# jonH34400/3DBodyAnimation

Hardware: AMD Instinct MI355X
Metric: SMPL residual+Jacobian evals/sec (6890v, 10 beta, 24 joints) (higher is better)
Workload: dtype f64 residual/Jacobian; f32 mesh (f32 + split-bf16 MFMA blend); 1 GPU; C3: 256 independent frames per GPU, BODY_25 (14 FK joints + 11 vertex landmarks), opt-shape (per-frame beta, 86 cols), GMM prior on, 6890-vertex mesh on; frames_per_gpu=256, keypoints_per_frame=25, n_cols=86

## Files before the change

### 3dbodyanimation_amd/csrc/frame_part_inl.h

```cpp
#pragma once
#include <hip/hip_ext.h>

#include "bodyfit_device.h"
#include "priors_inl.h"

namespace bodyfit {
namespace {

__device__ __forceinline__ void store_through(double* p, double v) {
  __hip_atomic_store(p, v, __ATOMIC_RELAXED, __HIP_MEMORY_SCOPE_SYSTEM);
}
#ifndef BODYFIT_J_THROUGH
#define BODYFIT_J_THROUGH 1
#endif
template <bool kFused>
__device__ __forceinline__ void store_J(double* p, double v, int scope = 0) {
  if constexpr (kFused && !BODYFIT_J_THROUGH) *p = v;
  else if (scope == 1) store_f64_through(p, v);
  else if (scope == 2) *p = v;
  else store_through(p, v);
}


__device__ inline void mul33(const double* A, const double* B, double* C) {
#pragma unroll
  for (int r = 0; r < 3; ++r)
#pragma unroll
    for (int c = 0; c < 3; ++c) C[r * 3 + c] = A[r * 3] * B[c] + A[r * 3 + 1] * B[3 + c] + A[r * 3 + 2] * B[6 + c];
}
__device__ inline void mul33_bt(const double* A, const double* B, double* C) {
#pragma unroll
  for (int r = 0; r < 3; ++r)
#pragma unroll
    for (int c = 0; c < 3; ++c)
      C[r * 3 + c] = A[r * 3] * B[c * 3] + A[r * 3 + 1] * B[c * 3 + 1] + A[r * 3 + 2] * B[c * 3 + 2];
}
__device__ inline void mv3(const double* A, double x0, double x1, double x2, double* y) {
#pragma unroll
  for (int r = 0; r < 3; ++r) y[r] = A[r * 3] * x0 + A[r * 3 + 1] * x1 + A[r * 3 + 2] * x2;
}

__device__ void rodrigues_grad_k(double a0, double a1, double a2, int k, double* R, double* dRk) {
  const double th2 = a0 * a0 + a1 * a1 + a2 * a2;
  if (th2 > 2.220446049250313e-16) {
    const double th = sqrt(th2), ith = 1.0 / th;
    double sh, ch;
    sincos(0.5 * th, &sh, &ch);
    const double st = 2.0 * sh * ch, omc = 2.0 * sh * sh, ct = 1.0 - omc;
    const double w[3] = {a0 * ith, a1 * ith, a2 * ith};
    const double K[9] = {0, -w[2], w[1], w[2], 0, -w[0], -w[1], w[0], 0};
#pragma unroll
    for (int r = 0; r < 3; ++r)
#pragma unroll
      for (int c = 0; c < 3; ++c) R[r * 3 + c] = (r == c ? ct : 0.0) + st * K[r * 3 + c] + omc * w[r] * w[c];
    const double wk = (k == 0) ? w[0] : (k == 1 ? w[1] : w[2]);
    double dw[3];
#pragma unroll
    for (int i = 0; i < 3; ++i) dw[i] = ((i == k ? 1.0 : 0.0) - w[i] * wk) * ith;
    const double dK[9] = {0, -dw[2], dw[1], dw[2], 0, -dw[0], -dw[1], dw[0], 0};
#pragma unroll
    for (int r = 0; r < 3; ++r)
#pragma unroll
      for (int c = 0; c < 3; ++c)
        dRk[r * 3 + c] = (r == c ? -st * wk : 0.0) + ct * wk * K[r * 3 + c] + st * dK[r * 3 + c] +
                         st * wk * w[r] * w[c] + omc * (dw[r] * w[c] + w[r] * dw[c]);
  } else {
    R[0] = 1; R[1] = -a2; R[2] = a1;
    R[3] = a2; R[4] = 1; R[5] = -a0;
    R[6] = -a1; R[7] = a0; R[8] = 1;
#pragma unroll
    for (int i = 0; i < 9; ++i) dRk[i] = 0.0;
    if (k == 0) { dRk[5] = -1; dRk[7] = 1; }
    else if (k == 1) { dRk[2] = 1; dRk[6] = -1; }
    else { dRk[1] = -1; dRk[3] = 1; }
  }
}

__device__ inline double wave_sum(double v) {
#pragma unroll
  for (int off = 32; off > 0; off >>= 1) v += __shfl_down(v, off, 64);
  return v;
}

#ifdef BODYFIT_STAMPS
#define STAMP(i)                                                                              \
  do {                                                                                        \
    if (Pb.dbg && (threadIdx.x & 63) == 0) {                                                  \
      unsigned long long t_;                                                                  \
      asm volatile("s_memtime %0\n\ts_waitcnt lgkmcnt(0)" : "=s"(t_)::"memory");              \
      Pb.dbg[((size_t)f * 8 + (threadIdx.x >> 6)) * 16 + (i)] = t_;                  \
    }                                                                                         \
  } while (0)
#define STAMP_REAL(i)                                                                         \
  do {                                                                                        \
    if (Pb.dbg && (threadIdx.x & 63) == 0) {                                                  \
      unsigned long long t_;                                                                  \
      asm volatile("s_memrealtime %0\n\ts_waitcnt lgkmcnt(0)" : "=s"(t_)::"memory");          \
      Pb.dbg[((size_t)f * 8 + (threadIdx.x >> 6)) * 16 + (i)] = t_;                  \
    }                                                                                         \
  } while (0)
#else
#define STAMP(i)
#define STAMP_REAL(i)
#endif

constexpr int KC = 32;
constexpr int kThreads = 512;

constexpr int OFF_X = 0;
constexpr int OFF_R = OFF_X + 88;
constexpr int OFF_DR = OFF_R + 216;
constexpr int OFF_A = OFF_DR + 648;
constexpr int OFF_P = OFF_A + 216;
constexpr int OFF_O = OFF_P + 72;
constexpr int OFF_JC = OFF_O + 72;
constexpr int OFF_W = OFF_JC + 72;
constexpr int OFF_B = OFF_W + 624;
constexpr int OFF_FEAT = OFF_B + 720;
constexpr int OFF_CAM = OFF_FEAT + 208;
constexpr int OFF_KP = OFF_CAM + 40;
constexpr int OFF_TAB = OFF_KP + KC * 18;
constexpr int OFF_KPUV = OFF_TAB + 64;
constexpr int OFF_DS = OFF_KPUV + 2 * KC;
constexpr int OFF_SC = OFF_DS + 720;
constexpr int OFF_PART = OFF_SC + 720;
constexpr int OFF_T = OFF_PART + 128;
constexpr int OFF_CHAIN = OFF_T + 720;
constexpr int OFF_LM = OFF_CHAIN + 24;
constexpr int LM_VP = 0;
constexpr int LM_Q = 3;
constexpr int LM_A = 6;
constexpr int LM_X = 15;
constexpr int LM_W = 39;
constexpr int LM_J = 47;
constexpr int LM_NW = 51;
constexpr int LM_BETA = 52;
constexpr int LM_PD = 82;
constexpr int LM_STRIDE = 290;
constexpr int TAB_PARENT = 0;
constexpr int TAB_ANC = 24;
constexpr int TAB_KPID = 96;

struct FrameHead {
  const unsigned char* mtab;
  const unsigned char* ptab;
  const double* R0;
  int F, K;
  int dims;
};
static_assert(kMaxJoints < 64 && kMaxShape < 16 && kMaxLandmarks < 64 && 7 + 3 * (kMaxJoints - 1) + kMaxShape < 256,
              "FrameHead::dims: 6 + 4 + 6 + 8 bits for nJ, nS, nL, ncols; beta_stride (0 or nS) in 4");
__host__ __device__ inline int frame_head_dims(int nJ, int nS, int nL, int ncols, int use_shape, int beta_stride, int has_coef) {
  return nJ | (nS << 6) | (nL << 10) | (ncols << 16) | ((use_shape ? 1 : 0) << 24) | (beta_stride << 25) | ((has_coef ? 1 : 0) << 29);
}

struct FusedFrame {
  unsigned* flag;
  unsigned epoch;
  int j_scope;
};

template <bool kFused>
__device__ __forceinline__ void frame_sync() {
  if constexpr (kFused) asm volatile("s_waitcnt lgkmcnt(0)\n\ts_barrier" ::: "memory");
  else __syncthreads();
}

template <bool kFused>
__device__ __forceinline__ void store_operand16(void* p, uint4 v) {
  if constexpr (kFused) {
    typedef __attribute__((ext_vector_type(4))) unsigned int u32x4_;
    const u32x4_ x = {v.x, v.y, v.z, v.w};
    asm volatile("global_store_dwordx4 %0, %1, off sc1\n\ts_nop 1" ::"v"(p), "v"(x) : "memory");
  } else {
    *reinterpret_cast<uint4*>(p) = v;
  }
}

template <bool kFused>
__device__ __forceinline__ void frame_part(const DevModel& M, const DevProblem& Pb, const double* __restrict__ params,
                                           const double* __restrict__ beta, double* __restrict__ r_out,
                                           double* __restrict__ J_out, double* __restrict__ joints_out, const MeshCoef& mc,
                                           int want_jac, double* sm, int f, const FusedFrame& fu, const FrameHead& hd) {
  const int tid = threadIdx.x;
  const int lane = tid & 63, wave = tid >> 6;
  const int nJ = kFused ? (hd.dims & 63) : M.nJ, nS = kFused ? ((hd.dims >> 6) & 15) : M.nS, nL = kFused ? ((hd.dims >> 10) & 63) : M.nL;
  const int ncols = kFused ? ((hd.dims >> 16) & 255) : Pb.ncols;
  const int npose = 7 + 3 * (nJ - 1);
  const bool use_shape = kFused ? (((hd.dims >> 24) & 1) != 0) : (Pb.use_shape != 0);
  const int beta_stride = kFused ? ((hd.dims >> 25) & 15) : Pb.beta_stride;
  const unsigned char* const mtab = kFused ? hd.mtab : M.tabA;
  const unsigned char* const ptab = kFused ? hd.ptab : Pb.ptab;
  const int* const t_parent = reinterpret_cast<const int*>(mtab + kTabParent);
  const unsigned* const t_anc = reinterpret_cast<const unsigned*>(mtab + kTabAnc);
  const unsigned long long* const t_chain = reinterpret_cast<const unsigned long long*>(mtab + kTabChain);
  const int* const t_lm_woff = reinterpret_cast<const int*>(mtab + kTabLmWoff);
  const int* const t_lm_wj = reinterpret_cast<const int*>(mtab + kTabLmWj);
  const double* const t_lm_ww = reinterpret_cast<const double*>(mtab + kTabLmWw);
  const double* const t_lm_vt = reinterpret_cast<const double*>(mtab + kTabLmVt);
  const double* const t_lm_sd = reinterpret_cast<const double*>(mtab + kTabLmSd);
  const double* const t_dS = reinterpret_cast<const double*>(mtab + kTabDS);
  const double* const t_Sc = reinterpret_cast<const double*>(mtab + kTabSc);
  const double* const t_offset = reinterpret_cast<const double*>(mtab + kTabOffset);
  const double* const t_Jc0 = reinterpret_cast<const double*>(mtab + kTabJc0);
  const int t_F = kFused ? hd.F : Pb.F, t_K = kFused ? hd.K : Pb.K;
  const int* const t_kp_offset = reinterpret_cast<const int*>(ptab);
  const int* const t_kp_id = reinterpret_cast<const int*>(ptab + ptab_id_off(t_F));
  const double* const t_kp_uv = reinterpret_cast<const double*>(ptab + ptab_uv_off(t_F, t_K));
  const double* const t_R0 = kFused ? hd.R0 : Pb.R0;
  const int P = M.P;
  double* sx = sm + OFF_X;
  double* sR = sm + OFF_R;
  double* sdR = sm + OFF_DR;
  double* sA = sm + OFF_A;
  double* sP = sm + OFF_P;
  double* sO = sm + OFF_O;
  double* sJc = sm + OFF_JC;
  double* sW = sm + OFF_W;
  double* sB = sm + OFF_B;
  double* sFeat = sm + OFF_FEAT;
  double* sCam = sm + OFF_CAM;
  double* sKp = sm + OFF_KP;
  int* sTab = reinterpret_cast<int*>(sm + OFF_TAB);
  double* sKpUv = sm + OFF_KPUV;
  double* sDS = sm + OFF_DS;
  double* sSc = sm + OFF_SC;
  double* sPart = sm + OFF_PART;
  double* sLm = sm + OFF_LM;
  double* sT = sm + OFF_T;
  double* sLmSd = sLm + nL * LM_STRIDE;
  int* sParent = sTab + TAB_PARENT;
  unsigned* sAnc = reinterpret_cast<unsigned*>(sTab + TAB_ANC);
  int* sKpId = sTab + TAB_KPID;
  unsigned* sKpAnc = reinterpret_cast<unsigned*>(sTab + 48);
  unsigned long long* sChain = reinterpret_cast<unsigned long long*>(sm + OFF_CHAIN);

  STAMP_REAL(10);
  STAMP(0);
#ifdef BODYFIT_STAMPS
  if (Pb.dbg && tid == 0) {
    unsigned xcc;
    asm volatile("s_getreg_b32 %0, hwreg(HW_REG_XCC_ID)" : "=s"(xcc));
    Pb.dbg[((size_t)f * 8) * 16 + 9] = xcc & 0xf;
  }
#endif
  if constexpr (!kFused) {
    if (Pb.frame_flags && !(Pb.frame_flags[f] & Pb.frame_mask)) return;
  }
  constexpr int kLoaders = kThreads;
  constexpr bool loader = true;
  constexpr int kSdPasses = (kMaxLandmarks * 3 * kMaxShape + kThreads - 1) / kThreads;
  constexpr int kPasses = (720 + kLoaders - 1) / kLoaders;
  const bool coef_wave = kFused && wave == 5 && ((hd.dims >> 29) & 1) != 0;
  const int tj_c = min(tid, nJ - 1);
  const int par_in = t_parent[tj_c];
  const unsigned anc_in = t_anc[tj_c];
  const unsigned long long chain_in = t_chain[tj_c];
  const int nlw = nL * kMaxLmNnz, lw_i = min(tid, max(nlw, 1) - 1);
  const double lww_in = t_lm_ww[lw_i];
  const int lwj_in = t_lm_wj[lw_i];
  const int lwo_in = t_lm_woff[lw_i / kMaxLmNnz];
  const int nsd = nL * 3 * nS, nds = nJ * 3 * nS;
  double sd_in[kSdPasses], t0[kPasses], t1[kPasses];
#pragma unroll
  for (int u = 0; u < kSdPasses; ++u) sd_in[u] = t_lm_sd[min(tid + u * kThreads, max(nsd, 1) - 1)];
#pragma unroll
  for (int u = 0; u < kPasses; ++u) {
    const int i = min(tid + u * kLoaders, max(nds, 1) - 1);
    t0[u] = t_dS[i];
    t1[u] = t_Sc[i];
  }
  const int k_begin0 = t_kp_offset[f], nk0 = min(KC, t_kp_offset[f + 1] - k_begin0);
  const int o_i = tid - 128, v_row = tid - 256;
  const bool o_lane = tid >= 128 && o_i < nJ * 3, v_lane = tid >= 256 && v_row < nL * 3;
  double o_pre = 0.0, jc_pre = 0.0, vt_pre = 0.0;
  if (o_lane) { o_pre = t_offset[o_i]; jc_pre = t_Jc0[o_i]; }
  if (v_lane) vt_pre = t_lm_vt[v_row];
  const int cam_lane = tid - 384;
  const bool cam_on = cam_lane >= 0 && cam_lane < 36;
  double r0c0 = 0.0, r0c1 = 0.0, r0c2 = 0.0;
  if (cam_on) {
    const double* R0 = t_R0 + (size_t)f * 9;
    const int c = cam_lane % 3;
    r0c0 = R0[c]; r0c1 = R0[3 + c]; r0c2 = R0[6 + c];
  }
  double x_in = 0.0;
  const bool x_lane = tid >= 128 && tid - 128 < npose, b_lane = tid >= 224 && tid - 224 < nS;
  if (x_lane) x_in = params[(size_t)f * npose + tid - 128];
  if (b_lane) x_in = (use_shape && beta) ? beta[(size_t)f * beta_stride + tid - 224] : 0.0;
  int kp_id0 = 0;
  double kp_u0 = 0.0, kp_v0 = 0.0;
  if (loader) {
    kp_id0 = t_kp_id[k_begin0 + (tid & (KC - 1))];
    kp_u0 = t_kp_uv[2 * (size_t)(k_begin0 + (tid & (KC - 1)))];
    kp_v0 = t_kp_uv[2 * (size_t)(k_begin0 + (tid & (KC - 1))) + 1];
  }
  if (tid < nJ) { sParent[tid] = par_in; sAnc[tid] = anc_in; sChain[tid] = chain_in; }
  volatile int* sWalkDone = reinterpret_cast<volatile int*>(sPart + 104);
  if (tid == 0) *sWalkDone = 0;
  if (tid < nlw) {
    const int l = tid / kMaxLmNnz, i = tid % kMaxLmNnz;
    double* L = sLm + l * LM_STRIDE;
    L[LM_W + i] = lww_in;
    reinterpret_cast<int*>(L + LM_J)[i] = lwj_in;
    if (i == 0) L[LM_NW] = (double)lwo_in;
  }
#pragma unroll
  for (int u = 0; u < kSdPasses; ++u)
    if (tid + u * kThreads < nsd) sLmSd[tid + u * kThreads] = sd_in[u];
#pragma unroll
  for (int u = 0; u < kPasses; ++u) {
    const int i = tid + u * kLoaders;
    if (i < nds) { sDS[i] = t0[u]; sSc[i] = t1[u]; }
  }
  if (x_lane) sx[tid - 128] = x_in;
  if (b_lane) sx[npose + tid - 224] = x_in;
  frame_sync<kFused>();
  if (tid < nk0) {
    sTab[TAB_KPID + tid] = kp_id0;
    sKpUv[2 * tid] = kp_u0;
    sKpUv[2 * tid + 1] = kp_v0;
  }
  const double* sbeta = sx + npose;

  STAMP(1);
  if (tid < 3 * nJ) {
    const int jj = tid / 3, k = tid - 3 * jj;
    const double* aa = (jj == 0) ? (sx + 1) : (sx + 7 + 3 * (jj - 1));
    double R[9], dRk[9];
    rodrigues_grad_k(aa[0], aa[1], aa[2], k, R, dRk);
    if (k == 0) {
#pragma unroll
      for (int i = 0; i < 9; ++i) sR[jj * 9 + i] = R[i];
    }
#pragma unroll
    for (int i = 0; i < 9; ++i) sdR[jj * 27 + k * 9 + i] = dRk[i];
  }
  if (v_lane) {
    const int row = v_row;
    double sv[kMaxShape];
#pragma unroll
    for (int k = 0; k < kMaxShape; ++k) sv[k] = (use_shape && k < nS) ? sLmSd[row * nS + k] : 0.0;
    double acc = vt_pre;
#pragma unroll
    for (int k = 0; k < kMaxShape; ++k) acc += sv[k] * sbeta[min(k, nS > 0 ? nS - 1 : 0)];
    sPart[row] = acc;
  }
  if (coef_wave) {
    float* cf = reinterpret_cast<float*>(sW);
    const int nfeat = 9 * (nJ - 1);
    if (lane < nJ - 1) {
      const float a0 = (float)sx[7 + 3 * lane], a1 = (float)sx[8 + 3 * lane], a2 = (float)sx[9 + 3 * lane];
      const float th2 = a0 * a0 + a1 * a1 + a2 * a2;
      float st = 1.0f, omc = 0.0f, w0 = a0, w1 = a1, w2 = a2;
      if (th2 > 1e-20f) {
        const float ith = rsqrtf(th2), th = th2 * ith;
        float sh, ch;
        sincosf(0.5f * th, &sh, &ch);
        st = 2.0f * sh * ch; omc = 2.0f * sh * sh;
        w0 = a0 * ith; w1 = a1 * ith; w2 = a2 * ith;
      }
      const float on = Pb.pose_blend ? 1.0f : 0.0f;
      float* o = cf + 9 * lane;
      o[0] = on * (omc * (w0 * w0 - 1.0f)); o[1] = on * (omc * w0 * w1 - st * w2); o[2] = on * (omc * w0 * w2 + st * w1);
      o[3] = on * (omc * w1 * w0 + st * w2); o[4] = on * (omc * (w1 * w1 - 1.0f)); o[5] = on * (omc * w1 * w2 - st * w0);
      o[6] = on * (omc * w2 * w0 - st * w1); o[7] = on * (omc * w2 * w1 + st * w0); o[8] = on * (omc * (w2 * w2 - 1.0f));
    } else if (lane >= 32 && lane - 32 < 16 * kBlendKSteps - kPoseFeat) {
      const int i = lane - 32;
      cf[kPoseFeat + i] = (i < nS) ? (float)sbeta[i] : ((i == kMaxShape || i == kMaxShape + 1) ? 1.0f : 0.0f);
    }
    if (lane < 32)
      for (int k = nfeat + lane; k < kPoseFeat; k += 32) cf[k] = 0.0f;
  }
  if (o_lane) {
    const int i = o_i;
    double o = o_pre, jc = jc_pre;
    if (use_shape) {
      for (int k = 0; k < nS; ++k) {
        o += sDS[i * nS + k] * sbeta[k];
        jc += sSc[i * nS + k] * sbeta[k];
      }
    }
    sO[i] = (i < 3) ? 0.0 : o;
    if (i < 3) sPart[100 + i] = o;
    sJc[i] = jc;
  }
  __builtin_amdgcn_s_waitcnt(0x0F70);
  frame_sync<kFused>();

  STAMP(2);
  const int lm_k = lane & 31, lm_l = 2 * wave + (lane >> 5);
  const bool lm_blend = Pb.pose_blend && P > 0;
  auto lm_load = [&](int l, double (&pdv)[27]) {
    const double* row = M.lm_pd + (size_t)min(l, max(nL, 1) - 1) * 27 * 32 + lm_k;
#pragma unroll
    for (int ae = 0; ae < 27; ++ae) pdv[ae] = row[ae * 32];
  };
  auto lm_terms = [&](int l, const double (&pdv)[27]) {
    const int k = min(lm_k + 1, nJ - 1);
    const bool lm_on = l < nL, on = lm_on && lm_k < nJ - 1;
    const double onf = (lm_blend && on) ? 1.0 : 0.0;
    double part[3] = {0.0, 0.0, 0.0};
#pragma unroll
    for (int e = 0; e < 9; ++e) {
      const double fe = (sR[k * 9 + e] - ((e % 4 == 0) ? 1.0 : 0.0)) * onf;
#pragma unroll
      for (int a = 0; a < 3; ++a) part[a] += pdv[a * 9 + e] * fe;
    }
    if (want_jac) {
#pragma unroll
      for (int c = 0; c < 3; ++c) {
        const double* d = sdR + k * 27 + c * 9;
        double h[3] = {0.0, 0.0, 0.0};
#pragma unroll
        for (int e = 0; e < 9; ++e) {
          const double de = d[e] * onf;
#pragma unroll
          for (int a = 0; a < 3; ++a) h[a] += pdv[a * 9 + e] * de;
        }
        if (on) {
          double* o = sLm + l * LM_STRIDE + LM_PD + (3 * (k - 1) + c) * 3;
          o[0] = h[0]; o[1] = h[1]; o[2] = h[2];
        }
      }
    }
#pragma unroll
    for (int a = 0; a < 3; ++a) {
#pragma unroll
      for (int off = 16; off > 0; off >>= 1) part[a] += __shfl_xor(part[a], off, 32);
    }
    if (lm_on && lm_k == 0) {
#pragma unroll
      for (int a = 0; a < 3; ++a) sLm[l * LM_STRIDE + LM_VP + a] = sPart[l * 3 + a] + part[a];
    }
  };
  const bool lm_wave0 = 2 * wave < nL, lm_wave1 = 2 * wave + 16 < nL;
  if (tid < 9) sA[tid] = (tid % 4 == 0) ? 1.0 : 0.0;
  if (tid >= 16 && tid < 19) sP[tid - 16] = 0.0;
  if (tid >= 32 && tid - 32 < 3 * nS) { sB[tid - 32] = 0.0; sT[tid - 32] = 0.0; }
  if (wave == 0) {
    asm volatile("s_waitcnt lgkmcnt(0)" ::: "memory");
    if (lane == 0) __hip_atomic_fetch_add(const_cast<int*>(sWalkDone), 1, __ATOMIC_RELAXED, __HIP_MEMORY_SCOPE_WORKGROUP);
  }
  if (coef_wave) {
    const float* cf = reinterpret_cast<const float*>(sW);
    if (lane < kBlendKSteps * 4) {
      const int kstep = lane >> 2, h = (lane >> 1) & 1, hl = lane & 1;
      const float4 v0 = *reinterpret_cast<const float4*>(cf + 16 * kstep + 8 * h);
      const float4 v1 = *reinterpret_cast<const float4*>(cf + 16 * kstep + 8 * h + 4);
      const float x[8] = {v0.x, v0.y, v0.z, v0.w, v1.x, v1.y, v1.z, v1.w};
      uint32_t pk[4];
#pragma unroll
      for (int q = 0; q < 4; ++q) {
        uint16_t b[2];
#pragma unroll
        for (int t = 0; t < 2; ++t) {
          const uint16_t hi = f32_to_bf16(x[2 * q + t]);
          b[t] = hl == 0 ? hi : f32_to_bf16(x[2 * q + t] - bf16_to_f32(hi));
        }
        pk[q] = (uint32_t)b[0] | ((uint32_t)b[1] << 16);
      }
      const int ftile = f / kFTile, phi = f % kFTile;
      const int row = 8 * (phi >> 3) + 4 * (phi & 1) + ((phi >> 1) & 3);
      uint4* dst = reinterpret_cast<uint4*>(reinterpret_cast<unsigned char*>(mc.featA) + ((size_t)ftile * kBlendKSteps + kstep) * 2048 +
                                            feat_frag_off(h * 32 + row, hl));
      store_operand16<true>(dst, make_uint4(pk[0], pk[1], pk[2], pk[3]));
    }
    asm volatile("s_waitcnt vmcnt(0)" ::: "memory");
    STAMP_REAL(14);
    if (lane == 0)
      (void)__hip_atomic_fetch_add(fu.flag + (size_t)(f / kFTile) * kUnitCounterStride + kUnitCoefOffset, 1u, __ATOMIC_RELAXED,
                                   __HIP_MEMORY_SCOPE_AGENT);
  }
  double pdv0[27];
  if (lm_wave0) lm_load(lm_l, pdv0);
  for (int i = tid; i < 208; i += kThreads) {
    double v = 0.0;
    if (i < 9 * (nJ - 1)) v = sR[9 + i] - (((i % 9) % 4 == 0) ? 1.0 : 0.0);
    sFeat[i] = v;
  }
  auto walk = [&](int kind, int j, int sel, bool on) {
    j = on ? j : 1;
    const double* tab = (kind == 2) ? sDS : sO;
    const int stride = (kind == 2) ? nS : 1, off = (kind == 2) ? sel : 0;
    const double m = (kind == 0) ? 0.0 : 1.0;
    const double* ini = (kind == 0) ? (sR + j * 9 + sel) : (tab + (j * 3) * stride + off);
    const int istride = (kind == 0) ? 3 : stride;
    double v0 = ini[0], v1 = ini[istride], v2 = ini[2 * istride];
    unsigned long long ch = on ? sChain[j] : 0ull;
    int k = (int)(ch & 31ull);
    double Rc[9], oc[3];
    auto fetch = [&](int kk, double (&Rn)[9], double (&on_)[3]) {
#pragma unroll
      for (int e = 0; e < 9; ++e) Rn[e] = sR[kk * 9 + e];
#pragma unroll
      for (int a3 = 0; a3 < 3; ++a3) on_[a3] = tab[(kk * 3 + a3) * stride + off];
    };
    fetch(k, Rc, oc);
    while (k > 0) {
      ch >>= 5;
      const int kn = (int)(ch & 31ull);
      double Rn[9], on_[3];
      fetch(kn, Rn, on_);
      const double t0 = Rc[0] * v0 + Rc[1] * v1 + Rc[2] * v2 + m * oc[0];
      const double t1 = Rc[3] * v0 + Rc[4] * v1 + Rc[5] * v2 + m * oc[1];
      const double t2 = Rc[6] * v0 + Rc[7] * v1 + Rc[8] * v2 + m * oc[2];
      v0 = t0; v1 = t1; v2 = t2;
#pragma unroll
      for (int e = 0; e < 9; ++e) Rc[e] = Rn[e];
      oc[0] = on_[0]; oc[1] = on_[1]; oc[2] = on_[2];
      k = kn;
    }
    if (!on) return;
    if (kind == 0) { sA[j * 9 + sel] = v0; sA[j * 9 + 3 + sel] = v1; sA[j * 9 + 6 + sel] = v2; }
    else if (kind == 1) { sP[j * 3] = v0; sP[j * 3 + 1] = v1; sP[j * 3 + 2] = v2; }
    else {
      sB[(j * 3 + 0) * nS + sel] = v0; sB[(j * 3 + 1) * nS + sel] = v1; sB[(j * 3 + 2) * nS + sel] = v2;
      double c[3];
      mv3(sA + j * 9, sSc[(j * 3 + 0) * nS + sel], sSc[(j * 3 + 1) * nS + sel], sSc[(j * 3 + 2) * nS + sel], c);
      sT[(j * 3 + 0) * nS + sel] = v0 - c[0]; sT[(j * 3 + 1) * nS + sel] = v1 - c[1]; sT[(j * 3 + 2) * nS + sel] = v2 - c[2];
    }
  };
  if (!kFused && wave == 0 && mc.featA) {
    const int ftile = f / kFTile, phi = f % kFTile;
    const int row = Pb.feat_perm ? (8 * (phi >> 3) + 4 * (phi & 1) + ((phi >> 1) & 3)) : phi;
    if (lane >= 8 && lane - 8 < kBlendKSteps * 4) {
      const int wl = lane - 8;
      const int kstep = wl >> 2, h = (wl >> 1) & 1, hl = wl & 1;
      const int k0 = kstep * 16 + 8 * h;
      const int nfeat = 9 * (nJ - 1);
      double vr[8], vb[8];
#pragma unroll
      for (int u = 0; u < 8; ++u) {
        vr[u] = sR[9 + min(k0 + u, nfeat - 1)];
        vb[u] = sbeta[min(max(k0 + u - kPoseFeat, 0), max(nS, 1) - 1)];
      }
      uint32_t pk[4];
#pragma unroll
      for (int jj = 0; jj < 4; ++jj) {
        uint16_t b[2];
#pragma unroll
        for (int u = 0; u < 2; ++u) {
          const int k = k0 + 2 * jj + u;
          const float xr = (Pb.pose_blend && k < nfeat) ? (float)(vr[2 * jj + u] - (((k % 9) % 4 == 0) ? 1.0 : 0.0)) : 0.0f;
          const float xb = (k - kPoseFeat < nS) ? (float)vb[2 * jj + u]
                                                : ((k == kPoseFeat + kMaxShape || k == kPoseFeat + kMaxShape + 1) ? 1.0f : 0.0f);
          const float x = (k < kPoseFeat) ? xr : xb;
          const uint16_t hi = f32_to_bf16(x);
          b[u] = hl == 0 ? hi : f32_to_bf16(x - bf16_to_f32(hi));
        }
        pk[jj] = (uint32_t)b[0] | ((uint32_t)b[1] << 16);
      }
      uint4* dst = reinterpret_cast<uint4*>(reinterpret_cast<unsigned char*>(mc.featA) + ((size_t)ftile * kBlendKSteps + kstep) * 2048 +
                                            feat_frag_off(h * 32 + row, hl));
      store_operand16<kFused>(dst, make_uint4(pk[0], pk[1], pk[2], pk[3]));
    }
  }
  if (cam_on) {
    const int mtx = cam_lane / 9, e = cam_lane % 9, r = e / 3;
    const double* Lm = (mtx == 0) ? sR : (sdR + (mtx - 1) * 9);
    sCam[cam_lane] = Lm[r * 3] * r0c0 + Lm[r * 3 + 1] * r0c1 + Lm[r * 3 + 2] * r0c2;
  }
  {
    const int nA = 3 * (nJ - 1), nP = nJ - 1;
    const int nA6 = (nA + 1) / 2, nP6 = (nP + 1) / 2;
    if (wave == 6 || wave == 7) {
      const int a0 = wave == 6 ? 0 : nA6, na = wave == 6 ? nA6 : nA - nA6;
      const int p0 = wave == 6 ? 0 : nP6, np = wave == 6 ? nP6 : nP - nP6;
      const bool isA = lane < na, isP = !isA && lane - na < np;
      const int item = isA ? a0 + lane : p0 + (lane - na);
      walk(isA ? 0 : 1, isA ? 1 + item / 3 : 1 + item, isA ? item % 3 : 0, isA || isP);
    }
  }
  if (wave == 6) {
    asm volatile("s_waitcnt lgkmcnt(0)" ::: "memory");
    if (lane == 0) __hip_atomic_fetch_add(const_cast<int*>(sWalkDone), 256, __ATOMIC_RELAXED, __HIP_MEMORY_SCOPE_WORKGROUP);
  }
  if (wave == 7) {
    STAMP(13);
    for (int spin = 0; spin < (1 << 20) && *sWalkDone < 257; ++spin) __builtin_amdgcn_s_sleep(1);
    asm volatile("" ::: "memory");
    STAMP(14);
    const double s_ = sx[0];
    const double* Rr0_ = sCam;
    for (int it = lane; it < 3 * nJ; it += 64) {
      const int jj = it / 3, r = it - 3 * jj;
      const double* Aj = sA + jj * 9;
      const double a0 = Rr0_[r * 3], a1 = Rr0_[r * 3 + 1], a2 = Rr0_[r * 3 + 2];
      double q[3];
      mv3(Aj, sJc[jj * 3], sJc[jj * 3 + 1], sJc[jj * 3 + 2], q);
      const double p0 = sP[jj * 3], p1 = sP[jj * 3 + 1], p2 = sP[jj * 3 + 2];
      if (mc.skinT) {
        const double ra0 = a0 * Aj[0] + a1 * Aj[3] + a2 * Aj[6];
        const double ra1 = a0 * Aj[1] + a1 * Aj[4] + a2 * Aj[7];
        const double ra2 = a0 * Aj[2] + a1 * Aj[5] + a2 * Aj[8];
        const double tr = a0 * (p0 - q[0]) + a1 * (p1 - q[1]) + a2 * (p2 - q[2]);
        float4* T = reinterpret_cast<float4*>(mc.skinT + (size_t)f * nJ * 12) + it;
        store_operand16<kFused>(T, make_uint4(__float_as_uint((float)(s_ * ra0)), __float_as_uint((float)(s_ * ra1)),
                                              __float_as_uint((float)(s_ * ra2)), __float_as_uint((float)(s_ * tr + sx[4 + r]))));
      }
      if (joints_out) joints_out[(size_t)f * nJ * 3 + it] = s_ * (a0 * p0 + a1 * p1 + a2 * p2) + sx[4 + r];
    }
    STAMP(15);
    if constexpr (kFused) {
      asm volatile("s_waitcnt vmcnt(0)" ::: "memory");
      STAMP_REAL(9);
      if (lane == 0)
        (void)__hip_atomic_fetch_add(fu.flag + (size_t)(f / kFTile) * kUnitCounterStride, 1u, __ATOMIC_RELAXED, __HIP_MEMORY_SCOPE_AGENT);
      STAMP_REAL(12);
    }
  }
  if (lm_wave0) lm_terms(lm_l, pdv0);
  if (lm_wave1) {
    double pdv1[27];
    lm_load(lm_l + 16, pdv1);
    lm_terms(lm_l + 16, pdv1);
  }
  STAMP(3);
  frame_sync<kFused>();

  STAMP(4);
  if (use_shape && want_jac) {
    for (int it = tid - 192; it >= 0 && tid < 448 && it < nS * (nJ - 1); it += 256) walk(2, 1 + it / nS, it % nS, true);
  }
  if (want_jac && tid < 3 * (nJ - 1)) {
    const int k = 1 + tid / 3, c = tid % 3, p = sParent[k];
    double T1[9], T2[9], Wm[9];
    mul33_bt(sdR + k * 27 + c * 9, sR + k * 9, T1);
    mul33(sA + p * 9, T1, T2);
    mul33_bt(T2, sA + p * 9, Wm);
#pragma unroll
    for (int e = 0; e < 9; ++e) sW[tid * 9 + e] = Wm[e];
  }
  if (wave == 2 && lane < nL) {
    double* L = sLm + lane * LM_STRIDE;
    const int* Lj = reinterpret_cast<const int*>(L + LM_J);
    double q[3] = {0, 0, 0}, Ab[9] = {0, 0, 0, 0, 0, 0, 0, 0, 0};
    const int nw = (int)L[LM_NW];
    for (int i = 0; i < nw; ++i) {
      const int j = Lj[i];
      const double w = L[LM_W + i];
      double xj[3];
      mv3(sA + j * 9, L[LM_VP] - sJc[j * 3], L[LM_VP + 1] - sJc[j * 3 + 1], L[LM_VP + 2] - sJc[j * 3 + 2], xj);
#pragma unroll
      for (int a = 0; a < 3; ++a) {
        xj[a] += sP[j * 3 + a];
        q[a] += w * xj[a];
        L[LM_X + i * 3 + a] = xj[a];
      }
#pragma unroll
      for (int e = 0; e < 9; ++e) Ab[e] += w * sA[j * 9 + e];
    }
#pragma unroll
    for (int a = 0; a < 3; ++a) L[LM_Q + a] = q[a];
#pragma unroll
    for (int e = 0; e < 9; ++e) L[LM_A + e] = Ab[e];
  }
  if (wave == 2 && M.lm_gcount) {
    const int cnt = (lane < nL) ? M.lm_gcount[lane] : 0;
    if (cnt > 1) {
      double* L = sLm + lane * LM_STRIDE;
      double q0 = L[LM_Q], q1 = L[LM_Q + 1], q2 = L[LM_Q + 2];
      for (int i = 1; i < cnt; ++i) {
        const double* Li = L + i * LM_STRIDE;
        q0 += Li[LM_Q]; q1 += Li[LM_Q + 1]; q2 += Li[LM_Q + 2];
      }
      L[LM_Q] = q0; L[LM_Q + 1] = q1; L[LM_Q + 2] = q2;
    }
  }
  frame_sync<kFused>();
  const double s = sx[0];
  const double* Rr0 = sCam;
  const double* dRr0 = sCam + 9;

  const int k_begin = k_begin0, k_end = k_begin0 + (Pb.kp_offset[f + 1] - k_begin0);
  const bool fold = Pb.beta_partials != nullptr && want_jac && ncols > npose && nS == kMaxShape;
  auto stage_kp = [&](int tid, int kc0) {
    {
      const int kg = kc0 + tid;
      const bool first = kc0 == k_begin;
      const int id = first ? sKpId[tid] : Pb.kp_id[kg];
      const double u_obs = first ? sKpUv[2 * tid] : Pb.kp_uv[2 * (size_t)kg];
      const double v_obs = first ? sKpUv[2 * tid + 1] : Pb.kp_uv[2 * (size_t)kg + 1];
      sKpId[tid] = id;
      sKpAnc[tid] = (id < nJ) ? sAnc[id] : 0u;
      double q[3];
      if (id < nJ) {
        if (id == 0 || sParent[id] < 0) {
#pragma unroll
          for (int a = 0; a < 3; ++a) q[a] = sPart[100 + a];
        } else {
#pragma unroll
          for (int a = 0; a < 3; ++a) q[a] = sP[id * 3 + a];
        }
      } else {
#pragma unroll
        for (int a = 0; a < 3; ++a) q[a] = sLm[(id - nJ) * LM_STRIDE + LM_Q + a];
      }
      double z[3];
      mv3(Rr0, q[0], q[1], q[2], z);
      const double X0 = s * z[0] + sx[4], X1 = s * z[1] + sx[5], X2 = s * z[2] + sx[6];
      const double iz = 1.0 / X2;
      const double res0 = Pb.fx * X0 * iz + Pb.cx - u_obs, res1 = Pb.fy * X1 * iz + Pb.cy - v_obs;
      r_out[2 * (size_t)kg] = res0;
      r_out[2 * (size_t)kg + 1] = res1;
      if (fold) {
        const double sq = res0 * res0 + res1 * res1, d2 = Pb.huber * Pb.huber;
        const bool outl = Pb.huber > 0.0 && sq > d2;
        const double rt = sqrt(sq);
        sKpUv[2 * tid] = res0;
        sKpUv[2 * tid + 1] = res1;
        sFeat[tid] = outl ? sqrt(Pb.huber / rt) : 1.0;
        sFeat[KC + tid] = 0.5 * (outl ? 2.0 * Pb.huber * rt - d2 : sq);
      }
      double* kp = sKp + tid * 18;
      const double dpi[6] = {Pb.fx * iz, 0.0, -Pb.fx * X0 * iz * iz, 0.0, Pb.fy * iz, -Pb.fy * X1 * iz * iz};
#pragma unroll
      for (int a = 0; a < 3; ++a) { kp[a] = q[a]; kp[3 + a] = z[a]; }
#pragma unroll
      for (int i = 0; i < 6; ++i) kp[6 + i] = dpi[i];
#pragma unroll
      for (int rr = 0; rr < 2; ++rr)
#pragma unroll
        for (int c = 0; c < 3; ++c)
          kp[12 + rr * 3 + c] = s * (dpi[rr * 3] * Rr0[c] + dpi[rr * 3 + 1] * Rr0[3 + c] + dpi[rr * 3 + 2] * Rr0[6 + c]);
    }
  };
  STAMP(5);
  if (wave == 6 && lane < min(KC, k_end - k_begin)) stage_kp(lane, k_begin);
  if (nL > 0 && want_jac) {
    for (int l = lm_l; l < nL; l += 16) {
      if (lm_k < nJ - 1) {
        const int k = lm_k + 1;
        const double* L = sLm + l * LM_STRIDE;
        const double* Ab = L + LM_A;
        const int* Lj = reinterpret_cast<const int*>(L + LM_J);
        const int nw = (int)L[LM_NW];
        const double pk0 = sP[k * 3], pk1 = sP[k * 3 + 1], pk2 = sP[k * 3 + 2];
        double a0 = 0, a1 = 0, a2 = 0;
        for (int i = 0; i < nw; ++i) {
          const int j = Lj[i];
          if (j == k || ((sAnc[j] >> k) & 1u)) {
            const double w = L[LM_W + i];
            a0 += w * (L[LM_X + i * 3] - pk0);
            a1 += w * (L[LM_X + i * 3 + 1] - pk1);
            a2 += w * (L[LM_X + i * 3 + 2] - pk2);
          }
        }
#pragma unroll
        for (int c = 0; c < 3; ++c) {
          double* o = sLm + l * LM_STRIDE + LM_PD + (3 * lm_k + c) * 3;
          const double* Wm = sW + (3 * lm_k + c) * 9;
          double t[3];
          mv3(Ab, o[0], o[1], o[2], t);
          o[0] = t[0] + Wm[0] * a0 + Wm[1] * a1 + Wm[2] * a2;
          o[1] = t[1] + Wm[3] * a0 + Wm[4] * a1 + Wm[5] * a2;
          o[2] = t[2] + Wm[6] * a0 + Wm[7] * a1 + Wm[8] * a2;
        }
      }
    }
    if (use_shape) {
      for (int it = kThreads - 1 - tid; it < nL * nS; it += kThreads) {
        const int l = it / nS, k = it % nS;
        const double* L = sLm + l * LM_STRIDE;
        const int* Lj = reinterpret_cast<const int*>(L + LM_J);
        double d[3];
        mv3(L + LM_A, sLmSd[(l * 3 + 0) * nS + k], sLmSd[(l * 3 + 1) * nS + k], sLmSd[(l * 3 + 2) * nS + k], d);
#pragma unroll
        for (int i = 0; i < kMaxLmNnz; ++i) {
          const int j = Lj[i];
          const double w = L[LM_W + i];
          d[0] += w * sT[(j * 3 + 0) * nS + k]; d[1] += w * sT[(j * 3 + 1) * nS + k]; d[2] += w * sT[(j * 3 + 2) * nS + k];
        }
        double* o = sLm + l * LM_STRIDE + LM_BETA + k * 3;
        o[0] = d[0]; o[1] = d[1]; o[2] = d[2];
      }
    }
  }

  STAMP(6);
  if (M.lm_gcount && want_jac && nL > 0) {
    frame_sync<kFused>();
    constexpr int kWords = LM_PD + 207 - LM_BETA;
    static_assert(LM_PD == LM_BETA + 30, "LM_BETA and LM_PD are adjacent");
    for (int it = tid; it < nL * kWords; it += kThreads) {
      const int l = it / kWords, w = it - l * kWords;
      const int cnt = M.lm_gcount[l];
      if (cnt > 1) {
        double* o = sLm + l * LM_STRIDE + LM_BETA + w;
        double v = o[0];
        for (int i = 1; i < cnt; ++i) v += o[i * LM_STRIDE];
        o[0] = v;
      }
    }
  }
  double* sJb = sdR;
  double fold_acc = 0.0;
  typedef __attribute__((ext_vector_type(4))) double fold_d4;
  fold_d4 fold_gram = {0.0, 0.0, 0.0, 0.0};
  for (int kc0 = k_begin; kc0 < k_end; kc0 += KC) {
    const int nk = min(KC, k_end - kc0);
    frame_sync<kFused>();
    if (kc0 != k_begin) {
      if (tid < nk) stage_kp(tid, kc0);
      frame_sync<kFused>();
    }
    STAMP(7);
    if (want_jac) {
      const int njc = npose - 7;
      const int ngrp = kThreads / njc;
      if (tid < ngrp * njc) {
        const int g = tid / njc, kc = tid - g * njc, k = 1 + kc / 3;
        double Wm[9];
#pragma unroll
        for (int e9 = 0; e9 < 9; ++e9) Wm[e9] = sW[kc * 9 + e9];
        const double pk0 = sP[k * 3], pk1 = sP[k * 3 + 1], pk2 = sP[k * 3 + 2];
        for (int kk = g; kk < nk; kk += ngrp) {
          const int kg = kc0 + kk;
          const int id = sKpId[kk];
          const unsigned am = sKpAnc[kk];
          const double* kp = sKp + kk * 18;
          const double* G = kp + 12;
          double d0 = 0.0, d1 = 0.0, d2 = 0.0;
          if (id < nJ) {
            if ((am >> k) & 1u) {
              const double x0 = kp[0] - pk0, x1 = kp[1] - pk1, x2 = kp[2] - pk2;
              d0 = Wm[0] * x0 + Wm[1] * x1 + Wm[2] * x2;
              d1 = Wm[3] * x0 + Wm[4] * x1 + Wm[5] * x2;
              d2 = Wm[6] * x0 + Wm[7] * x1 + Wm[8] * x2;
            }
          } else {
            const double* o = sLm + (id - nJ) * LM_STRIDE + LM_PD + kc * 3;
            d0 = o[0]; d1 = o[1]; d2 = o[2];
          }
          store_J<kFused>(J_out + (size_t)(2 * kg) * ncols + 7 + kc, G[0] * d0 + G[1] * d1 + G[2] * d2, fu.j_scope);
          store_J<kFused>(J_out + (size_t)(2 * kg + 1) * ncols + 7 + kc, G[3] * d0 + G[4] * d1 + G[5] * d2, fu.j_scope);
        }
      }
      const int nsc = 7 + (ncols - npose);
      for (int e = tid; e < nk * nsc; e += kThreads) {
        const int kk = e / nsc, c = e - kk * nsc;
        const int kg = kc0 + kk;
        const int id = sKpId[kk];
        const double* kp = sKp + kk * 18;
        const double* G = kp + 12;
        double j0, j1;
        int col;
        if (c == 0) {
          col = 0;
          j0 = kp[6] * kp[3] + kp[7] * kp[4] + kp[8] * kp[5];
          j1 = kp[9] * kp[3] + kp[10] * kp[4] + kp[11] * kp[5];
        } else if (c < 4) {
          col = c;
          double t[3];
          mv3(dRr0 + (c - 1) * 9, kp[0], kp[1], kp[2], t);
          j0 = s * (kp[6] * t[0] + kp[7] * t[1] + kp[8] * t[2]);
          j1 = s * (kp[9] * t[0] + kp[10] * t[1] + kp[11] * t[2]);
        } else if (c < 7) {
          col = c;
          j0 = kp[6 + (c - 4)];
          j1 = kp[9 + (c - 4)];
        } else {
          const int k = c - 7;
          col = npose + k;
          double d0 = 0.0, d1 = 0.0, d2 = 0.0;
          if (use_shape) {
            if (id < nJ) {
              if (id == 0 || sParent[id] < 0) {
                d0 = sDS[(id * 3 + 0) * nS + k]; d1 = sDS[(id * 3 + 1) * nS + k]; d2 = sDS[(id * 3 + 2) * nS + k];
              } else {
                d0 = sB[(id * 3 + 0) * nS + k]; d1 = sB[(id * 3 + 1) * nS + k]; d2 = sB[(id * 3 + 2) * nS + k];
              }
            } else {
              const double* o = sLm + (id - nJ) * LM_STRIDE + LM_BETA + k * 3;
              d0 = o[0]; d1 = o[1]; d2 = o[2];
            }
          }
          j0 = G[0] * d0 + G[1] * d1 + G[2] * d2;
          j1 = G[3] * d0 + G[4] * d1 + G[5] * d2;
        }
        store_J<kFused>(J_out + (size_t)(2 * kg) * ncols + col, j0, fu.j_scope);
        store_J<kFused>(J_out + (size_t)(2 * kg + 1) * ncols + col, j1, fu.j_scope);
        if (fold && c >= 7) { sJb[(2 * kk) * kMaxShape + c - 7] = j0; sJb[(2 * kk + 1) * kMaxShape + c - 7] = j1; }
      }
    }
    if (fold) {
      frame_sync<kFused>();
      if (wave == 0) {
        const int col = lane & 15, kq = lane >> 4;
        for (int s0 = 0; s0 < (2 * nk + 3) / 4; s0 += 4) {
          double vv[4];
#pragma unroll
          for (int u = 0; u < 4; ++u) {
            const int row = 4 * (s0 + u) + kq;
            const bool on = row < 2 * nk;
            const double sw = on ? sFeat[row >> 1] : 0.0;
            const double x = (on && col < nS) ? sJb[row * kMaxShape + col] : ((on && col == 10) ? sKpUv[row] : 0.0);
            vv[u] = sw * x;
          }
#pragma unroll
          for (int u = 0; u < 4; ++u) fold_gram = __builtin_amdgcn_mfma_f64_16x16x4f64(vv[u], vv[u], fold_gram, 0, 0, 0);
        }
      } else if (tid == 64) {
        for (int kk = 0; kk < nk; ++kk) fold_acc += sFeat[KC + kk];
      }
    }
  }
  if (fold) {
    double* out = Pb.beta_partials + (size_t)f * kReducePartial;
    if (wave == 0) {
#pragma unroll
      for (int q = 0; q < 4; ++q) {
        const int gi = (lane >> 4) + 4 * q, gj = lane & 15;
        if (gi < 10 && gj >= gi && gj <= 10) {
          double* o = out + fold_slot_gram(gi, gj);
          if constexpr (kFused) store_f64_through(o, fold_gram[q]); else *o = fold_gram[q];
        }
      }
    } else if (tid == 64) {
      if constexpr (kFused) store_f64_through(out + fold_slot_cost(0), fold_acc); else out[fold_slot_cost(0)] = fold_acc;
    }
  }
  STAMP(8);
  STAMP_REAL(11);
}

constexpr size_t frame_lds_bytes(int nL) { return (size_t)(OFF_LM + nL * (LM_STRIDE + 3 * kMaxShape)) * sizeof(double); }

}
}
```

Before: 12.58 million evals/s.

## Compute shape-derivative chain via per-joint local terms and ancestor summation

Replaces the per-(joint, beta) sequential kinematic chain walk for shape derivatives with a two-phase scheme. Each lane first computes its local term A_parent·dS and stores it in shared memory, then sums the stored local terms of its ancestors in batches of four. Work is mapped one half-wave per shape column and one lane per joint. This removes the serial 3x3 matrix-vector chain per lane and the extra loads the general walk needed. It relies on the chain encoding giving ancestors ending in zero, and on LDS visibility within a wave enforced only by an lgkmcnt wait with no barrier.

```diff
diff --git a/3dbodyanimation_amd/csrc/frame_part_inl.h b/3dbodyanimation_amd/csrc/frame_part_inl.h
--- a/3dbodyanimation_amd/csrc/frame_part_inl.h
+++ b/3dbodyanimation_amd/csrc/frame_part_inl.h
@@ -481,11 +481,9 @@
   }
   auto walk = [&](int kind, int j, int sel, bool on) {
     j = on ? j : 1;
-    const double* tab = (kind == 2) ? sDS : sO;
-    const int stride = (kind == 2) ? nS : 1, off = (kind == 2) ? sel : 0;
     const double m = (kind == 0) ? 0.0 : 1.0;
-    const double* ini = (kind == 0) ? (sR + j * 9 + sel) : (tab + (j * 3) * stride + off);
-    const int istride = (kind == 0) ? 3 : stride;
+    const double* ini = (kind == 0) ? (sR + j * 9 + sel) : (sO + j * 3);
+    const int istride = (kind == 0) ? 3 : 1;
     double v0 = ini[0], v1 = ini[istride], v2 = ini[2 * istride];
     unsigned long long ch = on ? sChain[j] : 0ull;
     int k = (int)(ch & 31ull);
@@ -494,7 +492,7 @@
 #pragma unroll
       for (int e = 0; e < 9; ++e) Rn[e] = sR[kk * 9 + e];
 #pragma unroll
-      for (int a3 = 0; a3 < 3; ++a3) on_[a3] = tab[(kk * 3 + a3) * stride + off];
+      for (int a3 = 0; a3 < 3; ++a3) on_[a3] = sO[kk * 3 + a3];
     };
     fetch(k, Rc, oc);
     while (k > 0) {
@@ -513,13 +511,7 @@
     }
     if (!on) return;
     if (kind == 0) { sA[j * 9 + sel] = v0; sA[j * 9 + 3 + sel] = v1; sA[j * 9 + 6 + sel] = v2; }
-    else if (kind == 1) { sP[j * 3] = v0; sP[j * 3 + 1] = v1; sP[j * 3 + 2] = v2; }
-    else {
-      sB[(j * 3 + 0) * nS + sel] = v0; sB[(j * 3 + 1) * nS + sel] = v1; sB[(j * 3 + 2) * nS + sel] = v2;
-      double c[3];
-      mv3(sA + j * 9, sSc[(j * 3 + 0) * nS + sel], sSc[(j * 3 + 1) * nS + sel], sSc[(j * 3 + 2) * nS + sel], c);
-      sT[(j * 3 + 0) * nS + sel] = v0 - c[0]; sT[(j * 3 + 1) * nS + sel] = v1 - c[1]; sT[(j * 3 + 2) * nS + sel] = v2 - c[2];
-    }
+    else { sP[j * 3] = v0; sP[j * 3 + 1] = v1; sP[j * 3 + 2] = v2; }
   };
   if (!kFused && wave == 0 && mc.featA) {
     const int ftile = f / kFTile, phi = f % kFTile;
@@ -620,8 +612,35 @@
   frame_sync<kFused>();
 
   STAMP(4);
-  if (use_shape && want_jac) {
-    for (int it = tid - 192; it >= 0 && tid < 448 && it < nS * (nJ - 1); it += 256) walk(2, 1 + it / nS, it % nS, true);
+  if (use_shape && want_jac && tid >= 192) {
+    static_assert(kMaxJoints - 1 <= 32 && kMaxShape * 32 <= kThreads - 192, "one half-wave per shape column, one lane per joint");
+    const int b = (tid - 192) >> 5, j = 1 + (lane & 31);
+    if (b < nS && j < nJ) {
+      const double* Ap = sA + max(sParent[j], 0) * 9;
+      const double s0 = sDS[(j * 3 + 0) * nS + b], s1 = sDS[(j * 3 + 1) * nS + b], s2 = sDS[(j * 3 + 2) * nS + b];
+      double v[3];
+      mv3(Ap, s0, s1, s2, v);
+      unsigned long long ch = sChain[j];
+      sB[(j * 3 + 0) * nS + b] = v[0]; sB[(j * 3 + 1) * nS + b] = v[1]; sB[(j * 3 + 2) * nS + b] = v[2];
+      asm volatile("s_waitcnt lgkmcnt(0)" ::: "memory");
+      while (__any(ch != 0ull)) {
+        double t[4][3];
+#pragma unroll
+        for (int u = 0; u < 4; ++u) {
+          const int k = (int)(ch & 31ull);
+          ch >>= 5;
+#pragma unroll
+          for (int a = 0; a < 3; ++a) t[u][a] = sB[(k * 3 + a) * nS + b];
+        }
+#pragma unroll
+        for (int u = 0; u < 4; ++u) { v[0] += t[u][0]; v[1] += t[u][1]; v[2] += t[u][2]; }
+      }
+      double c[3];
+      mv3(sA + j * 9, sSc[(j * 3 + 0) * nS + b], sSc[(j * 3 + 1) * nS + b], sSc[(j * 3 + 2) * nS + b], c);
+      asm volatile("" ::: "memory");
+      sB[(j * 3 + 0) * nS + b] = v[0]; sB[(j * 3 + 1) * nS + b] = v[1]; sB[(j * 3 + 2) * nS + b] = v[2];
+      sT[(j * 3 + 0) * nS + b] = v[0] - c[0]; sT[(j * 3 + 1) * nS + b] = v[1] - c[1]; sT[(j * 3 + 2) * nS + b] = v[2] - c[2];
+    }
   }
   if (want_jac && tid < 3 * (nJ - 1)) {
     const int k = 1 + tid / 3, c = tid % 3, p = sParent[k];
```

After: 12.55 million evals/s. About the same (-0.2%).
